# deepqmc/deepqmc

Measured on AMD Instinct MI355X. Metric: walker*local-energy evals/sec (VMC step: n_sub Metropolis sub-steps + E_loc + energy reduction), higher is better.
Workload: dtype f32

## Files before the change

### deepqmc_amd/csrc/kernel_linear.hip

```cpp
#include "common.h"
#include "kernels.h"

namespace dqmc {

template <typename real> __device__ __forceinline__ void act_derivs(int act, real v, real& y, real& d1, real& d2) {
  if (act == 1) {
    y = r_tanh<real>(v);
    d1 = 1 - y * y;
    d2 = -2 * y * d1;
  } else if (act == 2) {
    const real s = 1 / (1 + r_exp<real>(-v));
    y = v * s;
    d1 = s * (1 + v * (1 - s));
    d2 = s * (1 - s) * (2 + v * (1 - 2 * s));
  } else if (act == 3) {
    const real av = v < 0 ? -v : v;
    const real e = r_exp<real>(-av);
    const real s = v >= 0 ? 1 / (1 + e) : e / (1 + e);
    y = (v > 0 ? v : (real)0) + (sizeof(real) == 4 ? (real)log1pf((float)e) : (real)log1p((double)e)) - (real)0.69314718055994530942;
    d1 = s;
    d2 = s * (1 - s);
  } else if (act == 4) {
    const real t = r_tanh<real>(v * (real)0.25);
    y = 1 + 2 * t;
    d1 = (1 - t * t) * (real)0.5;
    d2 = -t * (1 - t * t) * (real)0.25;
  } else {
    y = v; d1 = 1; d2 = 0;
  }
}

struct TileId { int bx, by; };
__device__ __forceinline__ TileId tile_of_block() {
  const int gx = (int)gridDim.x, gy = (int)gridDim.y;
  TileId t{(int)blockIdx.x, (int)blockIdx.y};
  if (gy == 1) return t;
  const int b = (int)blockIdx.y * gx + (int)blockIdx.x;
  const int full = gx >> 3, region = full * 8 * gy;
  if (b < region) {
    const int xcd = b & 7, s_ = b >> 3;
    t.by = s_ % gy;
    t.bx = (s_ / gy) * 8 + xcd;
  } else {
    const int r = b - region;
    t.by = r % gy;
    t.bx = full * 8 + r / gy;
  }
  return t;
}

__device__ __forceinline__ long uniform_off(long v) {
  const unsigned lo = (unsigned)__builtin_amdgcn_readfirstlane((int)(unsigned)(unsigned long long)v);
  const unsigned hi = (unsigned)__builtin_amdgcn_readfirstlane((int)(unsigned)((unsigned long long)v >> 32));
  return (long)(((unsigned long long)hi << 32) | lo);
}

template <int BN> struct BStride { static constexpr int v = ((BN + 16) % 32 == 16) ? BN + 16 : BN + 32; };

template <typename real> struct HbmSink {
  real* dst;
  const real* res;
  real res_scale;
  int ld_dst, ld_res, col0_dst, rpw_dst, r0_dst, rpw_res, r0_res, TP, nrows;
  long drow0[2], rrow0[2];
  __device__ __forceinline__ HbmSink(const LinArgs<real>& a)
      : dst(a.dst), res(a.res), res_scale(a.res_scale), ld_dst(a.ld_dst), ld_res(a.ld_res), col0_dst(a.col0_dst), rpw_dst(a.rpw_dst),
        r0_dst(a.r0_dst), rpw_res(a.rpw_res), r0_res(a.r0_res), TP(a.TP), nrows(a.nrows) {}
  __device__ __forceinline__ void rows(int g, long& d, long& r) const {
    const int b = g / nrows, rr = g - b * nrows;
    d = ((long)b * rpw_dst + r0_dst + rr) * TP;
    r = res ? ((long)b * rpw_res + r0_res + rr) * TP : 0;
  }
  __device__ __forceinline__ void group(int slot, int g) {
    long d, r;
    rows(g, d, r);
    if (slot) { drow0[1] = d; rrow0[1] = r; } else { drow0[0] = d; rrow0[0] = r; }
  }
  __device__ __forceinline__ real fetch_at(long rrow, int col, bool ok) const {
    if (res == nullptr || !ok) return (real)0;
    return res[rrow * ld_res + col0_dst + col];
  }
  __device__ __forceinline__ void put_at(long drow, int , int col, real o, real r, bool ok) {
    if (!ok) return;
    if (res != nullptr) o = (r + o) * res_scale;
    dst[drow * ld_dst + col0_dst + col] = o;
  }
  __device__ __forceinline__ real fetch(int slot, int t, int col, bool ok) const { return fetch_at((slot ? rrow0[1] : rrow0[0]) + t, col, ok); }
  __device__ __forceinline__ void put(int slot, int t, int tile_row, int col, real o, real r, bool ok) { put_at((slot ? drow0[1] : drow0[0]) + t, tile_row, col, o, r, ok); }
  static constexpr bool fills = false;
  real* udst; const real* ures;
  __device__ __forceinline__ void ugroup(int g, int col_w0) {
    const int b = g / nrows, rr = g - b * nrows;
    udst = dst + uniform_off(((long)b * rpw_dst + r0_dst + rr) * TP * ld_dst + col0_dst + col_w0);
    ures = res ? res + uniform_off(((long)b * rpw_res + r0_res + rr) * TP * ld_res + col0_dst + col_w0) : nullptr;
  }
  __device__ __forceinline__ real ufetch(int t, int c) const {
    return ures ? *reinterpret_cast<const real*>(reinterpret_cast<const char*>(ures) + (unsigned)((t * ld_res + c) * (int)sizeof(real))) : (real)0;
  }
  __device__ __forceinline__ void uput(int t, int , int c, real o, real r) {
    if (ures != nullptr) o = (r + o) * res_scale;
    *reinterpret_cast<real*>(reinterpret_cast<char*>(udst) + (unsigned)((t * ld_dst + c) * (int)sizeof(real))) = o;
  }
  unsigned udd, urd;
  __device__ __forceinline__ void ugroup2(int g, bool second, int col_w0) {
    ugroup(g, col_w0);
    udd = urd = 0;
    if (second) {
      const int b0 = g / nrows, rr0 = g - b0 * nrows, b1 = (g + 1) / nrows, rr1 = g + 1 - b1 * nrows;
      udd = (unsigned)__builtin_amdgcn_readfirstlane((int)((((long)(b1 - b0) * rpw_dst + (rr1 - rr0)) * TP * ld_dst) * (long)sizeof(real)));
      urd = (unsigned)__builtin_amdgcn_readfirstlane((int)((((long)(b1 - b0) * rpw_res + (rr1 - rr0)) * TP * ld_res) * (long)sizeof(real)));
    }
  }
  __device__ __forceinline__ real ufetch2(bool h, int t, int c) const {
    return ures ? *reinterpret_cast<const real*>(reinterpret_cast<const char*>(ures) + ((h ? urd : 0u) + (unsigned)((t * ld_res + c) * (int)sizeof(real)))) : (real)0;
  }
  __device__ __forceinline__ void uput2(bool h, int t, int , int c, real o, real r) {
    if (ures != nullptr) o = (r + o) * res_scale;
    *reinterpret_cast<real*>(reinterpret_cast<char*>(udst) + ((h ? udd : 0u) + (unsigned)((t * ld_dst + c) * (int)sizeof(real)))) = o;
  }
};
template <typename real> struct LdsSink {
  real* hs;
  int stride;
  __device__ __forceinline__ void rows(int, long& d, long& r) const { d = 0; r = 0; }
  __device__ __forceinline__ void group(int, int) {}
  __device__ __forceinline__ real fetch_at(long, int, bool) const { return (real)0; }
  __device__ __forceinline__ void put_at(long, int tile_row, int col, real o, real, bool ok) { hs[tile_row * stride + col] = ok ? o : (real)0; }
  __device__ __forceinline__ real fetch(int, int, int, bool) const { return (real)0; }
  __device__ __forceinline__ void put(int, int, int tile_row, int col, real o, real, bool ok) { put_at(0, tile_row, col, o, (real)0, ok); }
  static constexpr bool fills = true;
  int ucol;
  __device__ __forceinline__ void ugroup(int, int col_w0) { ucol = col_w0; }
  __device__ __forceinline__ real ufetch(int, int) const { return (real)0; }
  __device__ __forceinline__ void uput(int, int tile_row, int c, real o, real) { hs[tile_row * stride + ucol + c] = o; }
  __device__ __forceinline__ void ugroup2(int, bool, int col_w0) { ucol = col_w0; }
  __device__ __forceinline__ real ufetch2(bool, int, int) const { return (real)0; }
  __device__ __forceinline__ void uput2(bool, int, int tile_row, int c, real o, real) { hs[tile_row * stride + ucol + c] = o; }
};

template <typename real, int ACT> __device__ __forceinline__ real act_value(real v) {
  real y, d1, d2;
  act_derivs<real>(ACT, v, y, d1, d2);
  return y;
}

template <typename real, int MR, int NR, int ACT, typename Sink>
__device__ __forceinline__ void value_rows_epilogue(typename Mfma<real>::acc_t (&acc)[MR][NR], int nrows, int ld_pre, const real* bias,
                                                    int ldw, const real* pre, int col_w0, int wm, int n_groups, Sink& sink, int bx) {
  constexpr int BM = 64 * MR;
  const int lane = threadIdx.x & 63, cl = lane & 15;
  real bv[NR];
  bool col_ok[NR];
#pragma unroll
  for (int n = 0; n < NR; ++n) {
    const int col = col_w0 + n * 16 + cl;
    col_ok[n] = col < ldw;
    bv[n] = (bias != nullptr && col_ok[n]) ? bias[col] : (real)0;
  }
#pragma unroll
  for (int i = 0; i < MR; ++i)
#pragma unroll
    for (int r0 = 0; r0 < 4; r0 += 2) {
      bool m_ok[2];
      int b[2];
      long drow[2], rrow[2];
#pragma unroll
      for (int q = 0; q < 2; ++q) {
        const int m = bx * BM + wm * (16 * MR) + i * 16 + Mfma<real>::row_of(lane, r0 + q);
        m_ok[q] = m < n_groups;
        b[q] = (m_ok[q] ? m : 0) / nrows;
        sink.rows(m_ok[q] ? m : 0, drow[q], rrow[q]);
      }
      real rres[2][NR], rpre[2][NR];
#pragma unroll
      for (int q = 0; q < 2; ++q)
#pragma unroll
        for (int n = 0; n < NR; ++n) {
          const int col = col_w0 + n * 16 + cl;
          rres[q][n] = sink.fetch_at(rrow[q], col, col_ok[n] && m_ok[q]);
          rpre[q][n] = (pre != nullptr && col_ok[n]) ? pre[(long)b[q] * ld_pre + col] : (real)0;
        }
#pragma unroll
      for (int q = 0; q < 2; ++q) {
        const int tile_row = wm * (16 * MR) + i * 16 + Mfma<real>::row_of(lane, r0 + q);
#pragma unroll
        for (int n = 0; n < NR; ++n) {
          const int col = col_w0 + n * 16 + cl;
          real v = acc[i][n][r0 + q];
          if (pre != nullptr && col_ok[n]) v += rpre[q][n];
          if (bias != nullptr && col_ok[n]) v += bv[n];
          sink.put_at(drow[q], tile_row, col, act_value<real, ACT>(v), rres[q][n], col_ok[n] && m_ok[q]);
        }
      }
    }
}

template <typename real, int MR, int NR, int GPW, typename Sink>
__device__ __forceinline__ void lin_epilogue(typename Mfma<real>::acc_t (&acc)[MR][NR], const LinArgs<real>& a, const real* bias, int act,
                                             int ldw, const real* pre, int col_w0, int wm, int n_groups, Sink& sink, int bx,
                                             real* xch = nullptr) {
  constexpr bool HALF = GPW == -1;
  constexpr bool SPLIT = GPW == -2;
  constexpr int GB = GPW > 0 ? MR / GPW : 1;
  const int lane = threadIdx.x & 63, cl = lane & 15;
  if (HALF) {
    constexpr bool F32L = sizeof(real) == 4;
    const int wmu = __builtin_amdgcn_readfirstlane(wm);
    const int Tm1 = a.T - 1;
    const int q = lane >> 4;
    real bvh[NR];
    bool col_ok[NR];
#pragma unroll
    for (int n = 0; n < NR; ++n) {
      const int col = col_w0 + n * 16 + cl;
      col_ok[n] = col < ldw;
      bvh[n] = (bias != nullptr && col_ok[n]) ? bias[col] : (real)0;
    }
#pragma unroll
    for (int i = 0; i < MR; ++i) {
      const int g0 = ((bx * 4 + wmu) * MR + i) * 2;
      const bool ok0 = g0 < n_groups, ok1 = g0 + 1 < n_groups;
      if (!ok0) {
        if constexpr (Sink::fills) {
          sink.ugroup2(0, false, col_w0);
#pragma unroll
          for (int n = 0; n < NR; ++n)
#pragma unroll
            for (int rg = 0; rg < 4; ++rg) sink.uput2(false, 0, wm * (16 * MR) + i * 16 + Mfma<real>::row_of(lane, rg), n * 16 + cl, (real)0, (real)0);
        }
        continue;
      }
      sink.ugroup2(g0, ok1, col_w0);
      real rres[NR][4];
#pragma unroll
      for (int n = 0; n < NR; ++n)
#pragma unroll
        for (int rg = 0; rg < 4; ++rg) {
          const int row = Mfma<real>::row_of(lane, rg);
          const bool h = row >> 3;
          rres[n][rg] = (col_ok[n] && (!h || ok1)) ? sink.ufetch2(h, row & 7, n * 16 + cl) : (real)0;
        }
#pragma unroll
      for (int n = 0; n < NR; ++n) {
        real y[2], d1[2], d2S[2];
        if constexpr (F32L) {
          real v = __shfl(acc[i][n][0], (lane & 32) + cl, 64) + bvh[n];
          real s_part = 0;
#pragma unroll
          for (int rg = 0; rg < 4; ++rg) {
            const int tt = (4 * q + rg) & 7;
            const real x = acc[i][n][rg];
            if (tt > 0 && tt < Tm1) s_part += x * x;
          }
          const real S = s_part + __shfl_xor(s_part, 16, 64);
          real d2;
          act_derivs<real>(act, v, y[0], d1[0], d2);
          d2S[0] = d2 * S;
          y[1] = y[0]; d1[1] = d1[0]; d2S[1] = d2S[0];
        } else {
#pragma unroll
          for (int h = 0; h < 2; ++h) {
            const real v = __shfl(acc[i][n][2 * h], cl, 64) + bvh[n];
            real s_part = 0;
#pragma unroll
            for (int rg = 2 * h; rg < 2 * h + 2; ++rg) {
              const int tt = Mfma<real>::row_of(lane, rg) & 7;
              const real x = acc[i][n][rg];
              if (tt > 0 && tt < Tm1) s_part += x * x;
            }
            const real S = quad_sum<real>(s_part);
            real d2;
            act_derivs<real>(act, v, y[h], d1[h], d2);
            d2S[h] = d2 * S;
          }
        }
#pragma unroll
        for (int rg = 0; rg < 4; ++rg) {
          const int row = Mfma<real>::row_of(lane, rg), tt = row & 7;
          const bool h = row >> 3;
          const int hs_ = F32L ? 0 : (rg >> 1);
          const real x = acc[i][n][rg];
          real o = r_fma<real>(d1[hs_], x, tt == Tm1 ? d2S[hs_] : (real)0);
          if (tt == 0) o = y[hs_];
          if (tt > Tm1) o = 0;
          const bool ok = col_ok[n] && (!h || ok1);
          if constexpr (Sink::fills) sink.uput2(h, tt, wm * (16 * MR) + i * 16 + row, n * 16 + cl, ok ? o : (real)0, rres[n][rg]);
          else if (ok) sink.uput2(h, tt, wm * (16 * MR) + i * 16 + row, n * 16 + cl, o, rres[n][rg]);
        }
// ... 102 lines not shown
      }
      sink.ugroup(g, col_w0);
      if (pre != nullptr) {
        const real* pw = pre + uniform_off((long)(g / a.nrows) * a.TP * a.ld_pre + col_w0);
#pragma unroll
        for (int n = 0; n < NR; ++n) {
          if (col_ok[n]) {
#pragma unroll
            for (int tb = 0; tb < GB; ++tb)
#pragma unroll
              for (int rg = 0; rg < 4; ++rg) {
                const int t = tb * 16 + Mfma<real>::row_of(lane, rg);
                acc[gj * GB + tb][n][rg] += *reinterpret_cast<const real*>(reinterpret_cast<const char*>(pw) + (unsigned)((t * a.ld_pre + n * 16 + cl) * (int)sizeof(real)));
              }
          }
        }
      }
      real rall[HOIST ? NR : 1][HOIST ? GB : 1][4];
      if constexpr (HOIST) {
#pragma unroll
        for (int n = 0; n < NR; ++n)
#pragma unroll
          for (int tb = 0; tb < GB; ++tb)
#pragma unroll
            for (int rg = 0; rg < 4; ++rg)
              rall[n][tb][rg] = col_ok[n] ? sink.ufetch(tb * 16 + Mfma<real>::row_of(lane, rg), n * 16 + cl) : (real)0;
      }
#pragma unroll
      for (int n = 0; n < NR; ++n) {
        real v = __shfl(acc[gj * GB][n][0], cl, 64) + bv[n];
        real s_part = 0;
#pragma unroll
        for (int tb = 0; tb < GB; ++tb)
#pragma unroll
          for (int rg = 0; rg < 4; ++rg) {
            const int t = tb * 16 + Mfma<real>::row_of(lane, rg);
            const real x = acc[gj * GB + tb][n][rg];
            if (t >= 1 && t < Tm1) s_part += x * x;
          }
        const real S = quad_sum<real>(s_part);
        real y, d1, d2;
        act_derivs<real>(act, v, y, d1, d2);
        const real d2S = d2 * S;
        constexpr int FB = HOIST ? GB : (((sizeof(real) == 8 && GB > 2) || GB == 4) ? 2 : GB);
#pragma unroll
        for (int tb0 = 0; tb0 < GB; tb0 += FB) {
          real rres[FB][4];
#pragma unroll
          for (int tb = 0; tb < FB; ++tb)
#pragma unroll
            for (int rg = 0; rg < 4; ++rg) {
              if constexpr (HOIST) rres[tb][rg] = rall[n][tb][rg];
              else rres[tb][rg] = (tb0 + tb < GB && col_ok[n]) ? sink.ufetch((tb0 + tb) * 16 + Mfma<real>::row_of(lane, rg), n * 16 + cl) : (real)0;
            }
          if (Sink::fills || col_ok[n]) {
#pragma unroll
            for (int tb = tb0; tb < tb0 + FB && tb < GB; ++tb)
#pragma unroll
              for (int rg = 0; rg < 4; ++rg) {
                const int row = Mfma<real>::row_of(lane, rg);
                const int t = tb * 16 + row;
                const real x = acc[gj * GB + tb][n][rg];
                real o = r_fma<real>(d1, x, t == Tm1 ? d2S : (real)0);
                if (t == 0) o = y;
                if (t > Tm1) o = 0;
                if (Sink::fills && !col_ok[n]) o = 0;
                sink.uput(t, wm * (16 * MR) + (gj * GB + tb) * 16 + row, n * 16 + cl, o, rres[tb - tb0][rg]);
              }
          }
        }
      }
    }
  } else {
    switch (act) {
      case 1: value_rows_epilogue<real, MR, NR, 1>(acc, a.nrows, a.ld_pre, bias, ldw, pre, col_w0, wm, n_groups, sink, bx); break;
      case 2: value_rows_epilogue<real, MR, NR, 2>(acc, a.nrows, a.ld_pre, bias, ldw, pre, col_w0, wm, n_groups, sink, bx); break;
      case 3: value_rows_epilogue<real, MR, NR, 3>(acc, a.nrows, a.ld_pre, bias, ldw, pre, col_w0, wm, n_groups, sink, bx); break;
      case 4: value_rows_epilogue<real, MR, NR, 4>(acc, a.nrows, a.ld_pre, bias, ldw, pre, col_w0, wm, n_groups, sink, bx); break;
      default: value_rows_epilogue<real, MR, NR, 0>(acc, a.nrows, a.ld_pre, bias, ldw, pre, col_w0, wm, n_groups, sink, bx); break;
    }
  }
}

template <typename real, int MR, int NR, int GPW, int WN, bool CHAIN = false, int NR2 = 2, int BKX = 1>
__global__ void __launch_bounds__(256 * WN, GPW == -2 ? 2 : (GPW == 0 && NR == 4 && WN == 2 && MR * sizeof(real) == 16) ? 4 : 1) k_linear(const LinArgs<real> a) {
  constexpr int NT = 256 * WN;
  constexpr int BM = 64 * MR, BN = 16 * NR * WN, BK = 16 * BKX, BK2 = 16;
  constexpr int AS = BK + 2, BS = BStride<BN>::v;
  constexpr bool HALF = GPW == -1;
  constexpr bool SPLIT = GPW == -2;
  constexpr int GB = GPW > 0 ? MR / GPW : 1;
  constexpr int APT = MR / WN;
  constexpr int NBV = (BK * BN / 4 + NT - 1) / NT;
  constexpr int HS = CHAIN ? BN + 2 : 1;
  constexpr int BN2 = 16 * NR2, BS2 = BStride<BN2>::v;
  constexpr bool FRESH = sizeof(real) == 4 && GPW != 0 && MR <= 3;
  static_assert(MR % WN == 0, "MR must be a multiple of WN");
  static_assert(!CHAIN || WN == 1, "chained layers use one column tile");
  static_assert(!SPLIT || (!CHAIN && WN == 1 && 6 * NR * 16 <= BM * AS), "split groups: plain layers, one column tile per workgroup");
  typedef typename Mfma<real>::acc_t acc_t;
  constexpr int N_AB = BM * AS + BK * BS, N_H = CHAIN ? BM * HS : 0, N_MAIN = N_AB > N_H ? N_AB : N_H;
  __shared__ __attribute__((aligned(32))) real smem_lin[N_MAIN + (CHAIN ? BK2 * BS2 : 0)];
  real* const As = smem_lin;
  real* const Bs = smem_lin + BM * AS;
  real* const Hs = smem_lin;
  real* const Bs2 = smem_lin + N_MAIN;
  static_assert((BM * AS) % 4 == 0 && N_MAIN % 4 == 0, "16-byte (float) / 32-byte (double) aligned LDS tiles");

  const int tid = threadIdx.x, lane = tid & 63, wave = tid >> 6;
  const int wm = wave & 3, wn = wave >> 2;
  const int n_groups = a.B * a.nrows;
  const TileId tile = tile_of_block();
  const int bx = tile.bx;
  const int col_blk0 = tile.by * BN;

  int a_row[APT];
  int a_g[APT], a_t[APT];
  const int a_kq = tid & 3;
#pragma unroll
  for (int j = 0; j < APT; ++j) {
    const int row = (tid >> 2) + (NT / 4) * j;
    a_row[j] = row;
    int g, t;
    if (HALF) {
      const int w = row / (16 * MR), rb = (row >> 4) % MR;
      g = ((bx * 4 + w) * MR + rb) * 2 + ((row & 15) >> 3);
      t = row & 7;
    } else if (SPLIT) {
      const int w = row / (16 * MR), rb = (row >> 4) % MR;
      g = bx * 2 + (w >> 1);
      t = ((w & 1) * MR + rb) * 16 + (row & 15);
    } else if (GPW > 0) {
      const int w = row / (16 * MR), rb = (row >> 4) % MR;
      g = (bx * 4 + w) * GPW + rb / GB;
      t = (rb % GB) * 16 + (row & 15);
    } else {
      g = bx * BM + row;
      t = 0;
    }
    a_g[j] = g < n_groups ? g : -1;
    a_t[j] = t;
  }

  acc_t acc[MR][NR];
#pragma unroll
  for (int i = 0; i < MR; ++i)
#pragma unroll
    for (int j = 0; j < NR; ++j) acc[i][j] = acc_t{0, 0, 0, 0};

  for (int p = 0; p < a.n_pieces; ++p) {
    const LinPiece<real> pc = a.piece[p];
    const int w_row0 = pc.w_row;
    const real* a_src[APT];
#pragma unroll
    for (int j = 0; j < APT; ++j) {
      if (a_g[j] >= 0) {
        const int b = a_g[j] / a.nrows, rr = a_g[j] - b * a.nrows;
        const long srow = ((long)b * pc.rpw + pc.r0 + (pc.bcast ? 0 : rr)) * a.TP + a_t[j];
        a_src[j] = pc.src + srow * pc.ld;
      } else {
        a_src[j] = nullptr;
      }
    }
    const int n_chunks = (pc.K + BK - 1) / BK;
    Vec4<real> ra[APT][BKX];
    real rb_[NBV][4];
    auto load_chunk = [&](int kc) {
#pragma unroll
      for (int j = 0; j < APT; ++j)
#pragma unroll
        for (int x = 0; x < BKX; ++x) {
          const int k0 = kc * BK + 16 * x + 4 * a_kq;
          if (a_src[j] != nullptr && k0 < pc.K) ra[j][x] = *reinterpret_cast<const Vec4<real>*>(a_src[j] + k0);
          else ra[j][x] = Vec4<real>{{0, 0, 0, 0}};
        }
#pragma unroll
      for (int j = 0; j < NBV; ++j) {
        const int f = tid + NT * j;
        const int k = f / (BN / 4), n4 = f % (BN / 4);
        const int kk = kc * BK + k, col = col_blk0 + 4 * n4;
        Vec4<real> t{{0, 0, 0, 0}};
        if (f < BK * BN / 4 && kk < pc.K && col < a.ldw) t = *reinterpret_cast<const Vec4<real>*>(a.W + (long)(w_row0 + kk) * a.ldw + col);
#pragma unroll
        for (int x = 0; x < 4; ++x) rb_[j][x] = t.v[x];
      }
    };
    load_chunk(0);
    for (int kc = 0; kc < n_chunks; ++kc) {
      __syncthreads();
#pragma unroll
      for (int j = 0; j < APT; ++j)
#pragma unroll
        for (int x = 0; x < BKX; ++x) {
          Vec2<real>* dst = reinterpret_cast<Vec2<real>*>(&As[a_row[j] * AS + 16 * x + 4 * a_kq]);
          dst[0] = Vec2<real>{{ra[j][x].v[0], ra[j][x].v[1]}};
          dst[1] = Vec2<real>{{ra[j][x].v[2], ra[j][x].v[3]}};
        }
#pragma unroll
      for (int j = 0; j < NBV; ++j) {
        const int f = tid + NT * j;
        if (f < BK * BN / 4) {
          const int k = f / (BN / 4), n4 = f % (BN / 4);
          *reinterpret_cast<Vec4<real>*>(&Bs[k * BS + 4 * n4]) = Vec4<real>{{rb_[j][0], rb_[j][1], rb_[j][2], rb_[j][3]}};
        }
      }
      __syncthreads();
      if (kc + 1 < n_chunks) load_chunk(kc + 1);
      acc_t part[FRESH ? MR : 1][FRESH ? NR : 1];
      if (FRESH) {
#pragma unroll
        for (int i = 0; i < MR; ++i)
#pragma unroll
          for (int j = 0; j < NR; ++j) part[FRESH ? i : 0][FRESH ? j : 0] = acc_t{0, 0, 0, 0};
      }
#pragma unroll
      for (int kk = 0; kk < BK / 4; ++kk) {
        const int kcol = kk * 4 + (lane >> 4);
        real fa[MR], fb[NR];
#pragma unroll
        for (int i = 0; i < MR; ++i) fa[i] = As[(wm * (16 * MR) + i * 16 + (lane & 15)) * AS + kcol];
#pragma unroll
        for (int j = 0; j < NR; ++j) fb[j] = Bs[kcol * BS + wn * (16 * NR) + j * 16 + (lane & 15)];
#pragma unroll
        for (int i = 0; i < MR; ++i)
#pragma unroll
          for (int j = 0; j < NR; ++j) {
            if (FRESH) part[FRESH ? i : 0][FRESH ? j : 0] = Mfma<real>::run(fa[i], fb[j], part[FRESH ? i : 0][FRESH ? j : 0]);
            else acc[i][j] = Mfma<real>::run(fa[i], fb[j], acc[i][j]);
          }
      }
      if (FRESH) {
#pragma unroll
        for (int i = 0; i < MR; ++i)
#pragma unroll
          for (int j = 0; j < NR; ++j)
#pragma unroll
            for (int x = 0; x < 4; ++x) acc[i][j][x] += part[FRESH ? i : 0][FRESH ? j : 0][x];
      }
    }
  }

  if (!CHAIN) {
    HbmSink<real> sink(a);
    lin_epilogue<real, MR, NR, GPW>(acc, a, a.bias, a.act, a.ldw, a.pre, col_blk0 + wn * (16 * NR), wm, n_groups, sink, bx, As);
    return;
  }
  auto second_layer = [&](acc_t (&h)[MR][NR], const real* bias1, const real* W2, const real* bias2, const LinArgs<real>& out) {
    static_assert(BK2 * BN2 / 4 <= NT, "one W2 vector per thread and chunk");
    const int K2 = a.ldw;
    const int n_chunks2 = (K2 + BK2 - 1) / BK2;
    real w2r[NR][4];
#pragma unroll
    for (int kc = 0; kc < NR; ++kc) {
      const int k = tid / (BN2 / 4), n4 = tid % (BN2 / 4);
      const int kk = kc * BK2 + k, col = 4 * n4;
      Vec4<real> t{{0, 0, 0, 0}};
      if (tid < BK2 * BN2 / 4 && kc < n_chunks2 && kk < K2 && col < a.ldw2) t = *reinterpret_cast<const Vec4<real>*>(W2 + (long)kk * a.ldw2 + col);
#pragma unroll
      for (int x = 0; x < 4; ++x) w2r[kc][x] = t.v[x];
    }
    {
      __syncthreads();
      LdsSink<real> hsink{Hs, HS};
      lin_epilogue<real, MR, NR, GPW>(h, a, bias1, a.act, a.ldw, (const real*)nullptr, 0, wm, n_groups, hsink, bx);
    }
    acc_t acc2[MR][NR2];
#pragma unroll
    for (int i = 0; i < MR; ++i)
#pragma unroll
      for (int j = 0; j < NR2; ++j) acc2[i][j] = acc_t{0, 0, 0, 0};
#pragma unroll
    for (int kc = 0; kc < NR; ++kc) {
      if (kc < n_chunks2) {
      __syncthreads();
      if (tid < BK2 * BN2 / 4) {
        const int k = tid / (BN2 / 4), n4 = tid % (BN2 / 4);
        *reinterpret_cast<Vec4<real>*>(&Bs2[k * BS2 + 4 * n4]) = Vec4<real>{{w2r[kc][0], w2r[kc][1], w2r[kc][2], w2r[kc][3]}};
      }
      __syncthreads();
#pragma unroll
      for (int kk = 0; kk < 4; ++kk) {
        const int kcol = kk * 4 + (lane >> 4);
        real fa[MR], fb[NR2];
#pragma unroll
        for (int i = 0; i < MR; ++i) fa[i] = Hs[(wm * (16 * MR) + i * 16 + (lane & 15)) * HS + kc * BK2 + kcol];
#pragma unroll
        for (int j = 0; j < NR2; ++j) fb[j] = Bs2[kcol * BS2 + j * 16 + (lane & 15)];
#pragma unroll
        for (int i = 0; i < MR; ++i)
#pragma unroll
          for (int j = 0; j < NR2; ++j) acc2[i][j] = Mfma<real>::run(fa[i], fb[j], acc2[i][j]);
      }
      }
    }
    HbmSink<real> sink(out);
    lin_epilogue<real, MR, NR2, GPW>(acc2, out, bias2, a.act2, a.ldw2, (const real*)nullptr, 0, wm, n_groups, sink, bx);
  };
  second_layer(acc, a.bias, a.W2, a.bias2, a);
}

__device__ __forceinline__ void sched_fence() { __builtin_amdgcn_sched_barrier(0); }
template <int MR, int NR, int GPW, int WN, int NP>
__global__ void __launch_bounds__(256 * WN, (MR == 3 && WN == 1) ? 3 : 1) k_linear_bf(const LinArgs<float> a) {
  typedef float real;
  constexpr int NT = 256 * WN;
  constexpr int BM = 64 * MR, BN = 16 * NR * WN, BK = 32;
  constexpr int AS = BK + 2, BSTR = BN + 4;
  constexpr bool HALF = GPW == -1;
  constexpr int GB = GPW > 0 ? MR / GPW : 1;
  constexpr int APT = MR / WN;
  constexpr int NBI = ((BK / 2) * (BN / 4) + NT - 1) / NT;
  constexpr bool HOLD_A = MR <= NR;
  constexpr bool BF_FRESH = NP == 9;
  static_assert(MR % WN == 0, "MR must be a multiple of WN");
  typedef Mfma<float>::acc_t acc_t;
  HIP_DYNAMIC_SHARED(char, smem_raw)
  float* As = reinterpret_cast<float*>(smem_raw);
  uint32_t* Bs = reinterpret_cast<uint32_t*>(smem_raw + (size_t)BM * AS * 4);

  const int tid = threadIdx.x, lane = tid & 63, wave = tid >> 6;
  const int wm = wave & 3, wn = wave >> 2;
  const int n_groups = a.B * a.nrows;
  const TileId tile = tile_of_block();
  const int bx = tile.bx;
  const int col_blk0 = tile.by * BN;
  const int kg = lane >> 4, l15 = lane & 15;

  int a_row[APT], a_g[APT], a_t[APT];
  const int a_kq = tid & 3;
#pragma unroll
  for (int j = 0; j < APT; ++j) {
    const int row = (tid >> 2) + (NT / 4) * j;
    a_row[j] = row;
    int g, t;
    if (HALF) {
      const int w = row / (16 * MR), rb = (row >> 4) % MR;
      g = ((bx * 4 + w) * MR + rb) * 2 + ((row & 15) >> 3);
      t = row & 7;
    } else if (GPW > 0) {
      const int w = row / (16 * MR), rb = (row >> 4) % MR;
      g = (bx * 4 + w) * GPW + rb / GB;
      t = (rb % GB) * 16 + (row & 15);
    } else {
      g = bx * BM + row;
      t = 0;
    }
    a_g[j] = g < n_groups ? g : -1;
    a_t[j] = t;
  }

  acc_t acc[MR][NR];
#pragma unroll
  for (int i = 0; i < MR; ++i)
#pragma unroll
    for (int j = 0; j < NR; ++j) acc[i][j] = acc_t{0, 0, 0, 0};

  for (int p = 0; p < a.n_pieces; ++p) {
    const LinPiece<real> pc = a.piece[p];
    const int w_row0 = pc.w_row;
    const real* a_src[APT];
#pragma unroll
    for (int j = 0; j < APT; ++j) {
      if (a_g[j] >= 0) {
        const int b = a_g[j] / a.nrows, rr = a_g[j] - b * a.nrows;
        const long srow = ((long)b * pc.rpw + pc.r0 + (pc.bcast ? 0 : rr)) * a.TP + a_t[j];
        a_src[j] = pc.src + srow * pc.ld;
      } else {
        a_src[j] = nullptr;
      }
    }
    const int n_chunks = (pc.K + BK - 1) / BK;
    Vec4<real> ra[APT][2], rb_[NBI][2];
    auto load_chunk = [&](int kc) {
#pragma unroll
      for (int j = 0; j < APT; ++j)
#pragma unroll
        for (int x = 0; x < 2; ++x) {
          const int k0 = kc * BK + 16 * x + 4 * a_kq;
          if (a_src[j] != nullptr && k0 < pc.K) ra[j][x] = *reinterpret_cast<const Vec4<real>*>(a_src[j] + k0);
// ... 72 lines not shown
        for (int j = 0; j < NR; ++j) {
          BfFrag b0, b1, b2;
          read_b(j, b0, b1, b2);
          acc_t part[MR];
#pragma unroll
          for (int i = 0; i < MR; ++i) part[i] = BF_FRESH ? acc_t{0, 0, 0, 0} : acc[i][j];
          if (NP == 9) {
#pragma unroll
            for (int i = 0; i < MR; ++i) part[i] = mfma_bf16(fa[i][2], b2, part[i]);
#pragma unroll
            for (int i = 0; i < MR; ++i) part[i] = mfma_bf16(fa[i][2], b1, part[i]);
#pragma unroll
            for (int i = 0; i < MR; ++i) part[i] = mfma_bf16(fa[i][1], b2, part[i]);
          }
#pragma unroll
          for (int i = 0; i < MR; ++i) part[i] = mfma_bf16(fa[i][2], b0, part[i]);
#pragma unroll
          for (int i = 0; i < MR; ++i) part[i] = mfma_bf16(fa[i][1], b1, part[i]);
#pragma unroll
          for (int i = 0; i < MR; ++i) part[i] = mfma_bf16(fa[i][0], b2, part[i]);
#pragma unroll
          for (int i = 0; i < MR; ++i) part[i] = mfma_bf16(fa[i][1], b0, part[i]);
#pragma unroll
          for (int i = 0; i < MR; ++i) part[i] = mfma_bf16(fa[i][0], b1, part[i]);
#pragma unroll
          for (int i = 0; i < MR; ++i) part[i] = mfma_bf16(fa[i][0], b0, part[i]);
#pragma unroll
          for (int i = 0; i < MR; ++i) {
            if (BF_FRESH) {
#pragma unroll
              for (int x = 0; x < 4; ++x) acc[i][j][x] += part[i][x];
            } else {
              acc[i][j] = part[i];
            }
          }
          sched_fence();
        }
      } else {
        BfFrag fb[NR][3];
#pragma unroll
        for (int j = 0; j < NR; ++j) read_b(j, fb[j][0], fb[j][1], fb[j][2]);
#pragma unroll
        for (int i = 0; i < MR; ++i) {
          BfFrag a0, a1, a2;
          read_a(i, a0, a1, a2);
          acc_t part[NR];
#pragma unroll
          for (int j = 0; j < NR; ++j) part[j] = BF_FRESH ? acc_t{0, 0, 0, 0} : acc[i][j];
          if (NP == 9) {
#pragma unroll
            for (int j = 0; j < NR; ++j) part[j] = mfma_bf16(a2, fb[j][2], part[j]);
#pragma unroll
            for (int j = 0; j < NR; ++j) part[j] = mfma_bf16(a2, fb[j][1], part[j]);
#pragma unroll
            for (int j = 0; j < NR; ++j) part[j] = mfma_bf16(a1, fb[j][2], part[j]);
          }
#pragma unroll
          for (int j = 0; j < NR; ++j) part[j] = mfma_bf16(a2, fb[j][0], part[j]);
#pragma unroll
          for (int j = 0; j < NR; ++j) part[j] = mfma_bf16(a1, fb[j][1], part[j]);
#pragma unroll
          for (int j = 0; j < NR; ++j) part[j] = mfma_bf16(a0, fb[j][2], part[j]);
#pragma unroll
          for (int j = 0; j < NR; ++j) part[j] = mfma_bf16(a1, fb[j][0], part[j]);
#pragma unroll
          for (int j = 0; j < NR; ++j) part[j] = mfma_bf16(a0, fb[j][1], part[j]);
#pragma unroll
          for (int j = 0; j < NR; ++j) part[j] = mfma_bf16(a0, fb[j][0], part[j]);
#pragma unroll
          for (int j = 0; j < NR; ++j) {
            if (BF_FRESH) {
#pragma unroll
              for (int x = 0; x < 4; ++x) acc[i][j][x] += part[j][x];
            } else {
              acc[i][j] = part[j];
            }
          }
          sched_fence();
        }
      }
    }
  }
  HbmSink<real> sink(a);
  lin_epilogue<real, MR, NR, GPW>(acc, a, a.bias, a.act, a.ldw, a.pre, col_blk0 + wn * (16 * NR), wm, n_groups, sink, bx);
}

static bool bf_pays(const LinArgs<float>& a, int np) {
  long chunks = 0, ksteps = 0;
  for (int p = 0; p < a.n_pieces; ++p) { chunks += (a.piece[p].K + 31) / 32; ksteps += (a.piece[p].K + 3) / 4; }
  return a.cfg_bf != 0 && chunks * np * 16 + chunks * 12 < ksteps * 32;
}
template <int MR, int NR, int GPW, int WN> static void launch_bf(hipStream_t st, const LinArgs<float>& a, unsigned gx, unsigned gy) {
  constexpr int BM = 64 * MR, BN = 16 * NR * WN;
  constexpr size_t lds = (size_t)BM * 34 * 4 + (size_t)3 * 16 * (BN + 4) * 4;
  constexpr int NP = GPW == 0 ? 6 : 9;
  static bool attr_set = false;
  if (!attr_set) {
    (void)hipFuncSetAttribute(reinterpret_cast<const void*>(&k_linear_bf<MR, NR, GPW, WN, NP>), hipFuncAttributeMaxDynamicSharedMemorySize, (int)lds);
    attr_set = true;
  }
  hipLaunchKernelGGL(HIP_KERNEL_NAME(k_linear_bf<MR, NR, GPW, WN, NP>), dim3(gx, gy), dim3(256 * WN), lds, st, a);
}
template <typename real, int MR, int NR, int GPW, int WN> struct BfLaunch {
  static bool run(hipStream_t, const LinArgs<real>&, unsigned, unsigned) { return false; }
};
template <int MR, int NR, int GPW, int WN> struct BfLaunch<float, MR, NR, GPW, WN> {
  static bool run(hipStream_t st, const LinArgs<float>& a, unsigned gx, unsigned gy) {
    if (!bf_pays(a, GPW == 0 ? 6 : 9)) return false;
    if (a.cfg_bf >= 2 && !(GPW > 0 && ((MR == 3 && WN == 1) || MR == GPW))) return false;
    launch_bf<MR, NR, GPW, WN>(st, a, gx, gy);
    return true;
  }
};

template <typename real> static bool wide_chunks(const LinArgs<real>& a) {
  int kmax = 0;
  for (int p = 0; p < a.n_pieces; ++p) kmax = a.piece[p].K > kmax ? a.piece[p].K : kmax;
  const bool on = sizeof(real) == 4 ? (a.cfg_bkx == 2 || a.cfg_bkx == 4) : (a.cfg_bkx == 3 || a.cfg_bkx == 4);
  return on && kmax >= 32;
}
template <typename real, int MR, int NR, int GPW, int WN> static void launch_cfg(hipStream_t st, const LinArgs<real>& a) {
  constexpr int BM = 64 * MR, BN = 16 * NR * WN;
  const long n_groups = (long)a.B * a.nrows;
  const unsigned gx = GPW == -2 ? (unsigned)((n_groups + 1) / 2)
                      : GPW < 0 ? (unsigned)((n_groups + 8 * MR - 1) / (8 * MR))
                      : GPW > 0 ? (unsigned)((n_groups + 4 * GPW - 1) / (4 * GPW)) : (unsigned)((n_groups + BM - 1) / BM);
  const unsigned gy = (unsigned)((a.ldw + BN - 1) / BN);
  if (BfLaunch<real, MR, NR, GPW, WN>::run(st, a, gx, gy)) return;
  if (MR == 1 && WN == 1 && GPW != 0 && wide_chunks(a))
    hipLaunchKernelGGL(HIP_KERNEL_NAME(k_linear<real, MR, NR, GPW, WN, false, 2, (MR == 1 && WN == 1 && GPW != 0) ? 2 : 1>), dim3(gx, gy), dim3(256 * WN), 0, st, a);
  else
    hipLaunchKernelGGL(HIP_KERNEL_NAME(k_linear<real, MR, NR, GPW, WN>), dim3(gx, gy), dim3(256 * WN), 0, st, a);
}
template <typename real, int MR, int NR, int GPW, int WN> static void launch_cfg_plain(hipStream_t st, const LinArgs<real>& a) {
  static_assert(GPW > 0 && MR > 1, "one-wave Laplacian groups");
  const long n_groups = (long)a.B * a.nrows;
  const unsigned gx = (unsigned)((n_groups + 4 * GPW - 1) / (4 * GPW)), gy = (unsigned)((a.ldw + 16 * NR * WN - 1) / (16 * NR * WN));
  hipLaunchKernelGGL(HIP_KERNEL_NAME(k_linear<real, MR, NR, GPW, WN>), dim3(gx, gy), dim3(256 * WN), 0, st, a);
}
template <typename real, int MR, int NR, int GPW> static void launch_chain_cfg(hipStream_t st, const LinArgs<real>& a) {
  constexpr int BM = 64 * MR;
  const long n_groups = (long)a.B * a.nrows;
  const unsigned gx = GPW < 0 ? (unsigned)((n_groups + 8 * MR - 1) / (8 * MR))
                      : GPW > 0 ? (unsigned)((n_groups + 4 * GPW - 1) / (4 * GPW)) : (unsigned)((n_groups + BM - 1) / BM);
  if (MR == 1 && GPW != 0 && wide_chunks(a))
    hipLaunchKernelGGL(HIP_KERNEL_NAME(k_linear<real, MR, NR, GPW, 1, true, 2, (MR == 1 && GPW != 0) ? 2 : 1>), dim3(gx, 1), dim3(256), 0, st, a);
  else
    hipLaunchKernelGGL(HIP_KERNEL_NAME(k_linear<real, MR, NR, GPW, 1, true, 2>), dim3(gx, 1), dim3(256), 0, st, a);
}
template <typename real, int MR, int GPW> static void launch_chain_nr(hipStream_t st, const LinArgs<real>& a) {
  if (a.ldw > 32) launch_chain_cfg<real, MR, 4, GPW>(st, a);
  else if (a.ldw > 16) launch_chain_cfg<real, MR, 2, GPW>(st, a);
  else launch_chain_cfg<real, MR, 1, GPW>(st, a);
}
bool linear_chain_supported(int TP, int ldw_hidden, int ldw_out) {
  return (TP == 1 || TP == 8 || TP == 16 || TP == 32) && ldw_hidden <= 64 && ldw_out <= 32;
}
template <typename real> void launch_linear_chain(hipStream_t st, const LinArgs<real>& a) {
  switch (a.TP) {
    case 1: launch_chain_nr<real, 1, 0>(st, a); break;
    case 8: launch_chain_nr<real, 1, -1>(st, a); break;
    case 16: launch_chain_nr<real, 1, 1>(st, a); break;
    case 32: launch_chain_nr<real, 2, 1>(st, a); break;
    default: break;
  }
}

// ... 79 lines not shown
```

Before: 973,900.

## Give each lane adjacent output columns so epilogue loads and stores vectorize

Remaps which output columns each lane owns in the MFMA linear kernel: each lane now holds NR adjacent columns (cl*NR+n) instead of columns strided by 16. The B tile is read with the matching column permutation, and its LDS stride is re-padded to avoid bank conflicts. New epilogue paths for half-group and wave-group tiles load residuals and store outputs as wide row vectors instead of scalar accesses. Launch-bounds minimum-wave hints are also retuned per configuration, which may change register pressure and occupancy.

```diff
diff --git a/deepqmc_amd/csrc/kernel_linear.hip b/deepqmc_amd/csrc/kernel_linear.hip
--- a/deepqmc_amd/csrc/kernel_linear.hip
+++ b/deepqmc_amd/csrc/kernel_linear.hip
@@ -57,6 +57,18 @@
 
 template <int BN> struct BStride { static constexpr int v = ((BN + 16) % 32 == 16) ? BN + 16 : BN + 32; };
 
+template <int NR, bool ADJ> __device__ __forceinline__ constexpr int col_of(int n, int cl) { return ADJ ? cl * NR + n : n * 16 + cl; }
+template <typename real, int N> struct __attribute__((aligned((N * sizeof(real) >= 16) ? 16 : N * sizeof(real)))) RowVec { real v[N]; };
+template <typename real, int NR, int BN> struct BStrideAdj {
+  static constexpr int W = NR * (int)sizeof(real) / 4, E = (int)sizeof(real) / 4;
+  static constexpr int words = BN * E;
+  static constexpr int up64 = (words + 63) / 64 * 64;
+  static constexpr int v = NR == 1 ? BStride<BN>::v
+                         : W == 2 ? ((words % 64 <= 32 ? words / 64 * 64 + 32 : up64 + 32) / E)
+                         : W == 4 ? up64 / E
+                                  : (up64 + 4) / E;
+};
+
 template <typename real> struct HbmSink {
   real* dst;
   const real* res;
@@ -117,6 +129,35 @@
   __device__ __forceinline__ void uput2(bool h, int t, int , int c, real o, real r) {
     if (ures != nullptr) o = (r + o) * res_scale;
     *reinterpret_cast<real*>(reinterpret_cast<char*>(udst) + ((h ? udd : 0u) + (unsigned)((t * ld_dst + c) * (int)sizeof(real)))) = o;
+  }
+  template <int NR> static __device__ __forceinline__ void ldv(const char* p, unsigned off, real (&r)[NR]) {
+    const RowVec<real, NR> x = *reinterpret_cast<const RowVec<real, NR>*>(p + off);
+#pragma unroll
+    for (int n = 0; n < NR; ++n) r[n] = x.v[n];
+  }
+  template <int NR> __device__ __forceinline__ void stv(char* p, unsigned off, const real (&o)[NR], const real (&r)[NR]) const {
+    RowVec<real, NR> x;
+#pragma unroll
+    for (int n = 0; n < NR; ++n) x.v[n] = res != nullptr ? (r[n] + o[n]) * res_scale : o[n];
+    *reinterpret_cast<RowVec<real, NR>*>(p + off) = x;
+  }
+  template <int NR> static __device__ __forceinline__ void zero(real (&r)[NR]) {
+#pragma unroll
+    for (int n = 0; n < NR; ++n) r[n] = 0;
+  }
+  template <int NR> __device__ __forceinline__ void ufetchv(int t, int c, real (&r)[NR]) const {
+    if (ures) ldv<NR>(reinterpret_cast<const char*>(ures), (unsigned)((t * ld_res + c) * (int)sizeof(real)), r);
+    else zero<NR>(r);
+  }
+  template <int NR> __device__ __forceinline__ void uputv(int t, int , int c, const real (&o)[NR], const real (&r)[NR]) {
+    stv<NR>(reinterpret_cast<char*>(udst), (unsigned)((t * ld_dst + c) * (int)sizeof(real)), o, r);
+  }
+  template <int NR> __device__ __forceinline__ void ufetch2v(bool h, int t, int c, real (&r)[NR]) const {
+    if (ures) ldv<NR>(reinterpret_cast<const char*>(ures), (h ? urd : 0u) + (unsigned)((t * ld_res + c) * (int)sizeof(real)), r);
+    else zero<NR>(r);
+  }
+  template <int NR> __device__ __forceinline__ void uput2v(bool h, int t, int , int c, const real (&o)[NR], const real (&r)[NR]) {
+    stv<NR>(reinterpret_cast<char*>(udst), (h ? udd : 0u) + (unsigned)((t * ld_dst + c) * (int)sizeof(real)), o, r);
   }
 };
 template <typename real> struct LdsSink {
@@ -136,6 +177,22 @@
   __device__ __forceinline__ void ugroup2(int, bool, int col_w0) { ucol = col_w0; }
   __device__ __forceinline__ real ufetch2(bool, int, int) const { return (real)0; }
   __device__ __forceinline__ void uput2(bool, int, int tile_row, int c, real o, real) { hs[tile_row * stride + ucol + c] = o; }
+  template <int NR> __device__ __forceinline__ void stv(int tile_row, int col, const real (&o)[NR]) {
+    if constexpr (NR == 1) {
+      hs[tile_row * stride + col] = o[0];
+    } else {
+      Vec2<real>* d = reinterpret_cast<Vec2<real>*>(&hs[tile_row * stride + col]);
+#pragma unroll
+      for (int n = 0; n < NR; n += 2) d[n / 2] = Vec2<real>{{o[n], o[n + 1]}};
+    }
+  }
+  template <int NR> __device__ __forceinline__ void ufetchv(int, int, real (&r)[NR]) const {
+#pragma unroll
+    for (int n = 0; n < NR; ++n) r[n] = 0;
+  }
+  template <int NR> __device__ __forceinline__ void uputv(int, int tile_row, int c, const real (&o)[NR], const real (&)[NR]) { stv<NR>(tile_row, ucol + c, o); }
+  template <int NR> __device__ __forceinline__ void ufetch2v(bool, int, int, real (&r)[NR]) const { ufetchv<NR>(0, 0, r); }
+  template <int NR> __device__ __forceinline__ void uput2v(bool, int, int tile_row, int c, const real (&o)[NR], const real (&)[NR]) { stv<NR>(tile_row, ucol + c, o); }
 };
 
 template <typename real, int ACT> __device__ __forceinline__ real act_value(real v) {
@@ -195,15 +252,233 @@
     }
 }
 
+template <typename real, int MR, int NR, typename Sink>
+__device__ __forceinline__ void half_groups_adj(typename Mfma<real>::acc_t (&acc)[MR][NR], const LinArgs<real>& a, const real* bias, int act,
+                                                int ldw, int col_w0, int wm, int n_groups, Sink& sink, int bx) {
+  constexpr bool F32L = sizeof(real) == 4;
+  const int lane = threadIdx.x & 63, cl = lane & 15, c = cl * NR;
+  const int wmu = __builtin_amdgcn_readfirstlane(wm);
+  const int Tm1 = a.T - 1;
+  const int q = lane >> 4;
+  const bool c_ok = col_w0 + c < ldw;
+  real bvh[NR], zero[NR];
+#pragma unroll
+  for (int n = 0; n < NR; ++n) { bvh[n] = (bias != nullptr && c_ok) ? bias[col_w0 + c + n] : (real)0; zero[n] = 0; }
+#pragma unroll
+  for (int i = 0; i < MR; ++i) {
+    const int g0 = ((bx * 4 + wmu) * MR + i) * 2;
+    const bool ok0 = g0 < n_groups, ok1 = g0 + 1 < n_groups;
+    if (!ok0) {
+      if constexpr (Sink::fills) {
+        sink.ugroup2(0, false, col_w0);
+#pragma unroll
+        for (int rg = 0; rg < 4; ++rg) sink.template uput2v<NR>(false, 0, wm * (16 * MR) + i * 16 + Mfma<real>::row_of(lane, rg), c, zero, zero);
+      }
+      continue;
+    }
+    sink.ugroup2(g0, ok1, col_w0);
+    real rres[4][NR];
+#pragma unroll
+    for (int rg = 0; rg < 4; ++rg) {
+      const int row = Mfma<real>::row_of(lane, rg);
+      const bool h = row >> 3;
+      if (c_ok && (!h || ok1)) sink.template ufetch2v<NR>(h, row & 7, c, rres[rg]);
+      else {
+#pragma unroll
+        for (int n = 0; n < NR; ++n) rres[rg][n] = 0;
+      }
+    }
+#pragma unroll
+    for (int n = 0; n < NR; ++n) {
+      real y[2], d1[2], d2S[2];
+      if constexpr (F32L) {
+        real v = __shfl(acc[i][n][0], (lane & 32) + cl, 64) + bvh[n];
+        real s_part = 0;
+#pragma unroll
+        for (int rg = 0; rg < 4; ++rg) {
+          const int tt = (4 * q + rg) & 7;
+          const real x = acc[i][n][rg];
+          if (tt > 0 && tt < Tm1) s_part += x * x;
+        }
+        const real S = s_part + __shfl_xor(s_part, 16, 64);
+        real d2;
+        act_derivs<real>(act, v, y[0], d1[0], d2);
+        d2S[0] = d2 * S;
+        y[1] = y[0]; d1[1] = d1[0]; d2S[1] = d2S[0];
+      } else {
+#pragma unroll
+        for (int h = 0; h < 2; ++h) {
+          const real v = __shfl(acc[i][n][2 * h], cl, 64) + bvh[n];
+          real s_part = 0;
+#pragma unroll
+          for (int rg = 2 * h; rg < 2 * h + 2; ++rg) {
+            const int tt = Mfma<real>::row_of(lane, rg) & 7;
+            const real x = acc[i][n][rg];
+            if (tt > 0 && tt < Tm1) s_part += x * x;
+          }
+          const real S = quad_sum<real>(s_part);
+          real d2;
+          act_derivs<real>(act, v, y[h], d1[h], d2);
+          d2S[h] = d2 * S;
+        }
+      }
+#pragma unroll
+      for (int rg = 0; rg < 4; ++rg) {
+        const int row = Mfma<real>::row_of(lane, rg), tt = row & 7;
+        const bool h = row >> 3;
+        const int hs_ = F32L ? 0 : (rg >> 1);
+        const real x = acc[i][n][rg];
+        real o = r_fma<real>(d1[hs_], x, tt == Tm1 ? d2S[hs_] : (real)0);
+        if (tt == 0) o = y[hs_];
+        if (tt > Tm1) o = 0;
+        if (Sink::fills && !(c_ok && (!h || ok1))) o = 0;
+        acc[i][n][rg] = o;
+      }
+    }
+#pragma unroll
+    for (int rg = 0; rg < 4; ++rg) {
+      const int row = Mfma<real>::row_of(lane, rg), tt = row & 7;
+      const bool h = row >> 3;
+      const bool ok = c_ok && (!h || ok1);
+      real o[NR];
+#pragma unroll
+      for (int n = 0; n < NR; ++n) o[n] = acc[i][n][rg];
+      if (Sink::fills || ok) sink.template uput2v<NR>(h, tt, wm * (16 * MR) + i * 16 + row, c, o, rres[rg]);
+    }
+  }
+}
+
 template <typename real, int MR, int NR, int GPW, typename Sink>
+__device__ __forceinline__ void wave_groups_adj(typename Mfma<real>::acc_t (&acc)[MR][NR], const LinArgs<real>& a, const real* bias, int act,
+                                                int ldw, const real* pre, int col_w0, int wm, int n_groups, Sink& sink, int bx) {
+  constexpr int GB = MR / GPW;
+  constexpr bool HOIST = GB * NR * 4 * (int)(sizeof(real) / 4) <= 32;
+  constexpr int FB = HOIST ? GB : (((sizeof(real) == 8 && GB > 2) || GB == 4) ? 2 : GB);
+  constexpr int FBV = HOIST ? GB : (FB / NR > 0 ? FB / NR : 1);
+  const int lane = threadIdx.x & 63, cl = lane & 15, c = cl * NR;
+  const int wmu = __builtin_amdgcn_readfirstlane(wm);
+  const int Tm1 = a.T - 1;
+  const bool c_ok = col_w0 + c < ldw;
+  real bv[NR], zero[NR];
+#pragma unroll
+  for (int n = 0; n < NR; ++n) { bv[n] = (bias != nullptr && c_ok) ? bias[col_w0 + c + n] : (real)0; zero[n] = 0; }
+#pragma unroll
+  for (int gj = 0; gj < GPW; ++gj) {
+    const int g = (bx * 4 + wmu) * GPW + gj;
+    if (g >= n_groups) {
+      if constexpr (Sink::fills) {
+        sink.ugroup(0, col_w0);
+#pragma unroll
+        for (int tb = 0; tb < GB; ++tb)
+#pragma unroll
+          for (int rg = 0; rg < 4; ++rg)
+            sink.template uputv<NR>(0, wm * (16 * MR) + (gj * GB + tb) * 16 + Mfma<real>::row_of(lane, rg), c, zero, zero);
+      }
+      continue;
+    }
+    sink.ugroup(g, col_w0);
+    if (pre != nullptr && c_ok) {
+      const real* pw = pre + uniform_off((long)(g / a.nrows) * a.TP * a.ld_pre + col_w0);
+#pragma unroll
+      for (int tb = 0; tb < GB; ++tb)
+#pragma unroll
+        for (int rg = 0; rg < 4; ++rg) {
+          const int t = tb * 16 + Mfma<real>::row_of(lane, rg);
+          const RowVec<real, NR> x = *reinterpret_cast<const RowVec<real, NR>*>(reinterpret_cast<const char*>(pw) + (unsigned)((t * a.ld_pre + c) * (int)sizeof(real)));
+#pragma unroll
+          for (int n = 0; n < NR; ++n) acc[gj * GB + tb][n][rg] += x.v[n];
+        }
+    }
+    real rall[HOIST ? GB : 1][4][NR];
+    if constexpr (HOIST) {
+#pragma unroll
+      for (int tb = 0; tb < GB; ++tb)
+#pragma unroll
+        for (int rg = 0; rg < 4; ++rg) {
+          if (c_ok) sink.template ufetchv<NR>(tb * 16 + Mfma<real>::row_of(lane, rg), c, rall[tb][rg]);
+          else {
+#pragma unroll
+            for (int n = 0; n < NR; ++n) rall[tb][rg][n] = 0;
+          }
+        }
+    }
+#pragma unroll
+    for (int n = 0; n < NR; ++n) {
+      real v = __shfl(acc[gj * GB][n][0], cl, 64) + bv[n];
+      real s_part = 0;
+#pragma unroll
+      for (int tb = 0; tb < GB; ++tb)
+#pragma unroll
+        for (int rg = 0; rg < 4; ++rg) {
+          const int t = tb * 16 + Mfma<real>::row_of(lane, rg);
+          const real x = acc[gj * GB + tb][n][rg];
+          if (t >= 1 && t < Tm1) s_part += x * x;
+        }
+      const real S = quad_sum<real>(s_part);
+      real y, d1, d2;
+      act_derivs<real>(act, v, y, d1, d2);
+      const real d2S = d2 * S;
+#pragma unroll
+      for (int tb = 0; tb < GB; ++tb)
+#pragma unroll
+        for (int rg = 0; rg < 4; ++rg) {
+          const int t = tb * 16 + Mfma<real>::row_of(lane, rg);
+          const real x = acc[gj * GB + tb][n][rg];
+          real o = r_fma<real>(d1, x, t == Tm1 ? d2S : (real)0);
+          if (t == 0) o = y;
+          if (t > Tm1) o = 0;
+          if (Sink::fills && !c_ok) o = 0;
+          acc[gj * GB + tb][n][rg] = o;
+        }
+    }
+#pragma unroll
+    for (int tb0 = 0; tb0 < GB; tb0 += FBV) {
+      real rres[FBV][4][NR];
+#pragma unroll
+      for (int tb = 0; tb < FBV; ++tb)
+#pragma unroll
+        for (int rg = 0; rg < 4; ++rg) {
+          if constexpr (HOIST) {
+#pragma unroll
+            for (int n = 0; n < NR; ++n) rres[tb][rg][n] = rall[tb][rg][n];
+          } else {
+            if (tb0 + tb < GB && c_ok) sink.template ufetchv<NR>((tb0 + tb) * 16 + Mfma<real>::row_of(lane, rg), c, rres[tb][rg]);
+            else {
+#pragma unroll
+              for (int n = 0; n < NR; ++n) rres[tb][rg][n] = 0;
+            }
+          }
+        }
+      if (Sink::fills || c_ok) {
+#pragma unroll
+        for (int tb = tb0; tb < tb0 + FBV && tb < GB; ++tb)
+#pragma unroll
+          for (int rg = 0; rg < 4; ++rg) {
+            const int row = Mfma<real>::row_of(lane, rg);
+            real o[NR];
+#pragma unroll
+            for (int n = 0; n < NR; ++n) o[n] = acc[gj * GB + tb][n][rg];
+            sink.template uputv<NR>(tb * 16 + row, wm * (16 * MR) + (gj * GB + tb) * 16 + row, c, o, rres[tb - tb0][rg]);
+          }
+      }
+    }
+  }
+}
+
+template <typename real, int MR, int NR, int GPW, bool ADJ, typename Sink>
 __device__ __forceinline__ void lin_epilogue(typename Mfma<real>::acc_t (&acc)[MR][NR], const LinArgs<real>& a, const real* bias, int act,
                                              int ldw, const real* pre, int col_w0, int wm, int n_groups, Sink& sink, int bx,
                                              real* xch = nullptr) {
   constexpr bool HALF = GPW == -1;
   constexpr bool SPLIT = GPW == -2;
   constexpr int GB = GPW > 0 ? MR / GPW : 1;
+  static_assert(!(ADJ && SPLIT && NR > 1), "the split-group tiles keep the column-block mapping");
   const int lane = threadIdx.x & 63, cl = lane & 15;
-  if (HALF) {
+  if constexpr (ADJ && NR > 1 && HALF) {
+    half_groups_adj<real, MR, NR>(acc, a, bias, act, ldw, col_w0, wm, n_groups, sink, bx);
+  } else if constexpr (ADJ && NR > 1 && (GPW > 0)) {
+    wave_groups_adj<real, MR, NR, (GPW > 0 ? GPW : 1)>(acc, a, bias, act, ldw, pre, col_w0, wm, n_groups, sink, bx);
+  } else if (HALF) {
     constexpr bool F32L = sizeof(real) == 4;
     const int wmu = __builtin_amdgcn_readfirstlane(wm);
     const int Tm1 = a.T - 1;
@@ -472,18 +747,30 @@
   }
 }
 
+template <typename real, int MR, int NR, int GPW> constexpr bool lin_adj() {
+  return GPW != -2 && GPW != 0 && !(sizeof(real) == 8 && (MR >= 10 || (NR == 4 && GPW == -1)));
+}
+template <typename real, int MR, int NR, int GPW, int WN, bool CHAIN, int BKX> constexpr int lin_min_waves() {
+  if (GPW == -2) return 2;
+  if (GPW == 0) return (NR == 4 && WN == 2 && MR * sizeof(real) == 16) ? 4 : 1;
+  if (MR == 1 && WN == 1 && sizeof(real) == 4) return NR == 2 ? ((CHAIN && BKX == 2) ? 7 : 8) : NR == 4 ? ((CHAIN && BKX == 2) ? 4 : 5) : 1;
+  if (MR == 1 && WN == 1 && sizeof(real) == 8) return NR == 4 ? (GPW == 1 ? 3 : 1) : (GPW == 1 && (NR == 2) != CHAIN) ? 5 : 1;
+  if (MR == 6 && NR == 2 && sizeof(real) == 8) return 2;
+  return 1;
+}
 template <typename real, int MR, int NR, int GPW, int WN, bool CHAIN = false, int NR2 = 2, int BKX = 1>
-__global__ void __launch_bounds__(256 * WN, GPW == -2 ? 2 : (GPW == 0 && NR == 4 && WN == 2 && MR * sizeof(real) == 16) ? 4 : 1) k_linear(const LinArgs<real> a) {
+__global__ void __launch_bounds__(256 * WN, (lin_min_waves<real, MR, NR, GPW, WN, CHAIN, BKX>())) k_linear(const LinArgs<real> a) {
   constexpr int NT = 256 * WN;
   constexpr int BM = 64 * MR, BN = 16 * NR * WN, BK = 16 * BKX, BK2 = 16;
-  constexpr int AS = BK + 2, BS = BStride<BN>::v;
   constexpr bool HALF = GPW == -1;
   constexpr bool SPLIT = GPW == -2;
+  constexpr bool ADJ = lin_adj<real, MR, NR, GPW>();
+  constexpr int AS = BK + 2, BS = ADJ ? BStrideAdj<real, NR, BN>::v : BStride<BN>::v;
   constexpr int GB = GPW > 0 ? MR / GPW : 1;
   constexpr int APT = MR / WN;
   constexpr int NBV = (BK * BN / 4 + NT - 1) / NT;
   constexpr int HS = CHAIN ? BN + 2 : 1;
-  constexpr int BN2 = 16 * NR2, BS2 = BStride<BN2>::v;
+  constexpr int BN2 = 16 * NR2, BS2 = ADJ ? BStrideAdj<real, NR2, BN2>::v : BStride<BN2>::v;
   constexpr bool FRESH = sizeof(real) == 4 && GPW != 0 && MR <= 3;
   static_assert(MR % WN == 0, "MR must be a multiple of WN");
   static_assert(!CHAIN || WN == 1, "chained layers use one column tile");
@@ -610,7 +897,7 @@
 #pragma unroll
         for (int i = 0; i < MR; ++i) fa[i] = As[(wm * (16 * MR) + i * 16 + (lane & 15)) * AS + kcol];
 #pragma unroll
-        for (int j = 0; j < NR; ++j) fb[j] = Bs[kcol * BS + wn * (16 * NR) + j * 16 + (lane & 15)];
+        for (int j = 0; j < NR; ++j) fb[j] = Bs[kcol * BS + wn * (16 * NR) + col_of<NR, ADJ>(j, lane & 15)];
 #pragma unroll
         for (int i = 0; i < MR; ++i)
 #pragma unroll
@@ -632,7 +919,7 @@
 
   if (!CHAIN) {
     HbmSink<real> sink(a);
-    lin_epilogue<real, MR, NR, GPW>(acc, a, a.bias, a.act, a.ldw, a.pre, col_blk0 + wn * (16 * NR), wm, n_groups, sink, bx, As);
+    lin_epilogue<real, MR, NR, GPW, ADJ>(acc, a, a.bias, a.act, a.ldw, a.pre, col_blk0 + wn * (16 * NR), wm, n_groups, sink, bx, As);
     return;
   }
   auto second_layer = [&](acc_t (&h)[MR][NR], const real* bias1, const real* W2, const real* bias2, const LinArgs<real>& out) {
@@ -652,7 +939,7 @@
     {
       __syncthreads();
       LdsSink<real> hsink{Hs, HS};
-      lin_epilogue<real, MR, NR, GPW>(h, a, bias1, a.act, a.ldw, (const real*)nullptr, 0, wm, n_groups, hsink, bx);
+      lin_epilogue<real, MR, NR, GPW, ADJ>(h, a, bias1, a.act, a.ldw, (const real*)nullptr, 0, wm, n_groups, hsink, bx);
     }
     acc_t acc2[MR][NR2];
 #pragma unroll
@@ -675,7 +962,7 @@
 #pragma unroll
         for (int i = 0; i < MR; ++i) fa[i] = Hs[(wm * (16 * MR) + i * 16 + (lane & 15)) * HS + kc * BK2 + kcol];
 #pragma unroll
-        for (int j = 0; j < NR2; ++j) fb[j] = Bs2[kcol * BS2 + j * 16 + (lane & 15)];
+        for (int j = 0; j < NR2; ++j) fb[j] = Bs2[kcol * BS2 + col_of<NR2, ADJ>(j, lane & 15)];
 #pragma unroll
         for (int i = 0; i < MR; ++i)
 #pragma unroll
@@ -684,7 +971,7 @@
       }
     }
     HbmSink<real> sink(out);
-    lin_epilogue<real, MR, NR2, GPW>(acc2, out, bias2, a.act2, a.ldw2, (const real*)nullptr, 0, wm, n_groups, sink, bx);
+    lin_epilogue<real, MR, NR2, GPW, ADJ>(acc2, out, bias2, a.act2, a.ldw2, (const real*)nullptr, 0, wm, n_groups, sink, bx);
   };
   second_layer(acc, a.bias, a.W2, a.bias2, a);
 }
@@ -923,7 +1210,7 @@
     }
   }
   HbmSink<real> sink(a);
-  lin_epilogue<real, MR, NR, GPW>(acc, a, a.bias, a.act, a.ldw, a.pre, col_blk0 + wn * (16 * NR), wm, n_groups, sink, bx);
+  lin_epilogue<real, MR, NR, GPW, false>(acc, a, a.bias, a.act, a.ldw, a.pre, col_blk0 + wn * (16 * NR), wm, n_groups, sink, bx);
 }
 
 static bool bf_pays(const LinArgs<float>& a, int np) {
```

Result: no change. 991,100, median of 6 (+1.8%).
